# alejandrofontan/AnyFeature-VSLAM

Hardware: AMD Instinct MI355X
Metric: keypoints extracted+matched /sec (ORB32, 640x480) (higher is better)
Workload: dtype u8; 1 GPU; ORB32 640x480 synthetic corners frames (LCG), 1000 kp/frame budget, 8 levels x1.2, FAST 20; extract+describe on device, brute-force Hamming match frame t vs t-1 (TH 75, ratio 0.6, orientation check); parallelism=frames sharded x1

## Files before the change

anyfeature-vslam_amd/csrc/k_harris.hip:

```cpp
#include <algorithm>

#include "afv_device.h"
#include "afv_wave.h"
#include "afv_runtime.h"

typedef short short2v __attribute__((ext_vector_type(2)));
typedef unsigned int uint2v __attribute__((ext_vector_type(2)));
typedef unsigned int uint3v __attribute__((ext_vector_type(3)));
__device__ __forceinline__ uint32_t as_u32(short2v v) { return __builtin_bit_cast(uint32_t, v); }
__device__ __forceinline__ short2v as_s2(uint32_t v) { return __builtin_bit_cast(short2v, v); }

#define RS_CPT 36
#define HQ_CHUNK 64

__device__ __forceinline__ int wave_incl_scan_shfl(int v) { return afv_wave_incl_scan(v); }

__global__ __launch_bounds__(256) void k_retain_score(const Geo *__restrict__ geo_p, const uint32_t *__restrict__ cand_packed,
                                                      const int *__restrict__ cand_count, uint32_t *__restrict__ l1,
                                                      int *__restrict__ l1_count, uint2 *__restrict__ queue, int *__restrict__ queue_n,
                                                      int frame_base, int total_blocks) {
    __shared__ int hist[256];
    __shared__ int wsum[4];
    __shared__ int s_T1, s_n1, s_qb;
    const Geo &geo = *geo_p;
    const int work = afv_xcd_remap(blockIdx.x, total_blocks);
    if (work >= total_blocks) return;
    const int l = work % geo.nlevels, f = frame_base + work / geo.nlevels;
    const LevelGeo &L = geo.lv[l];
    const size_t base = L.cand_off + (size_t)f * L.cand_frame_stride;
    const uint32_t *cp = cand_packed + base;
    uint32_t *out = l1 + base;
    const int n = min(cand_count[f * AFV_MAX_LEVELS + l], L.cand_cap);
    const int tid = threadIdx.x, lane = tid & 63;
    const int K = 2 * L.cv_quota;
    int n1 = n;
    const bool reg = n <= 256 * RS_CPT;
    uint32_t cpk[RS_CPT];
    if (reg) {
#pragma unroll
        for (int k = 0; k < RS_CPT; ++k) {
            cpk[k] = 0;
            if (k * 256 < n && k * 256 + tid < n) cpk[k] = cp[k * 256 + tid];
        }
    }
    if (n > K) {
        hist[tid] = 0;
        if (tid == 0) {
            s_T1 = 0;
            s_n1 = 0;
        }
        __syncthreads();
        if (reg) {
#pragma unroll
            for (int k = 0; k < RS_CPT; ++k)
                if (k * 256 < n && k * 256 + tid < n) atomicAdd(&hist[cpk[k] >> 24], 1);
        } else {
            for (int i = tid; i < n; i += 256) atomicAdd(&hist[cp[i] >> 24], 1);
        }
        __syncthreads();
        const int h = hist[255 - tid];
        const int incl = wave_incl_scan_shfl(h);
        if (lane == 63) wsum[tid >> 6] = incl;
        __syncthreads();
        int before = incl - h;
        for (int w = 0; w < (tid >> 6); ++w) before += wsum[w];
        if (before < K && K <= before + h) s_T1 = 255 - tid;
        __syncthreads();
        const int T1 = s_T1;
        auto emit = [&](bool in, uint32_t e) {
            const bool keep = in && (int)(e >> 24) >= T1;
            const unsigned long long m = __ballot(keep);
            int wbase = 0;
            if (lane == 0 && m) wbase = atomicAdd(&s_n1, __popcll(m));
            wbase = __shfl(wbase, 0, 64);
            if (keep) out[wbase + __popcll(m & ((1ull << lane) - 1ull))] = e;
        };
        if (reg) {
#pragma unroll
            for (int k = 0; k < RS_CPT; ++k) {
                if (k * 256 >= n) break;
                emit(k * 256 + tid < n, cpk[k]);
            }
        } else {
            for (int i0 = 0; i0 < n; i0 += 256) {
                const int i = i0 + tid;
                emit(i < n, i < n ? cp[i] : 0u);
            }
        }
        __syncthreads();
        n1 = s_n1;
    } else if (reg) {
#pragma unroll
        for (int k = 0; k < RS_CPT; ++k)
            if (k * 256 < n && k * 256 + tid < n) out[k * 256 + tid] = cpk[k];
    } else {
        for (int i = tid; i < n; i += 256) out[i] = cp[i];
    }
    const int nchunks = (n1 + HQ_CHUNK - 1) / HQ_CHUNK;
    if (tid == 0) {
        l1_count[f * AFV_MAX_LEVELS + l] = n1;
        s_qb = nchunks ? atomicAdd(queue_n, nchunks) : 0;
    }
    __syncthreads();
    const int qb = s_qb;
    for (int i = tid; i < nchunks; i += 256) queue[qb + i] = make_uint2((uint32_t)(f * AFV_MAX_LEVELS + l), (uint32_t)(i * HQ_CHUNK) | ((uint32_t)min(HQ_CHUNK, n1 - i * HQ_CHUNK) << 24));
}

struct HarrisItem {
    const uint8_t *img;
    __amdgpu_buffer_rsrc_t rsrc;
    int pitch, lw, lh, cnt;
    size_t base;
};

__device__ __forceinline__ void harris_item_rsrc(HarrisItem &it) {
    const uint64_t ip = reinterpret_cast<uint64_t>(it.img);
    const uint32_t ip_lo = (uint32_t)__builtin_amdgcn_readfirstlane((int)(uint32_t)ip), ip_hi = (uint32_t)__builtin_amdgcn_readfirstlane((int)(uint32_t)(ip >> 32));
    it.img = reinterpret_cast<const uint8_t *>(((uint64_t)ip_hi << 32) | ip_lo);
    it.pitch = __builtin_amdgcn_readfirstlane(it.pitch);
    it.lw = __builtin_amdgcn_readfirstlane(it.lw);
    it.lh = __builtin_amdgcn_readfirstlane(it.lh);
    it.rsrc = __builtin_amdgcn_make_buffer_rsrc(const_cast<uint8_t *>(it.img), 0, (it.lh - 1) * it.pitch + it.lw, 0x00027000);
}

__device__ __forceinline__ HarrisItem harris_item(const Geo &geo, const FrameSrc &src0, const uint8_t *pyr, uint2 item) {
    HarrisItem it;
    const int fl = (int)item.x, f = fl / AFV_MAX_LEVELS, l = fl - f * AFV_MAX_LEVELS;
    const LevelGeo &L = geo.lv[l];
    if (l == 0) {
        it.img = src0.base + (size_t)f * src0.frame_stride;
        it.pitch = src0.stride;
    } else {
        it.img = pyr + L.pyr_off + (size_t)f * L.pyr_frame_stride;
        it.pitch = L.pitch;
    }
    it.lw = L.w;
    it.lh = L.h;
    it.cnt = (int)(item.y >> 24);
    it.base = L.cand_off + (size_t)f * L.cand_frame_stride + (size_t)(item.y & 0x00ffffffu);
    harris_item_rsrc(it);
    return it;
}

__device__ __forceinline__ float harris_response(const HarrisItem &it, uint32_t e, float scale4) {
    const int px = (int)(e & 4095u), py = (int)((e >> 12) & 4095u);
    const bool left = px < 4, right = px + 4 >= it.lw;
    const int xa = left ? 0 : ((px - 4) & ~3), sh = left ? 0 : ((px - 4) & 3);
    const uint32_t selA = 0x0c010c00u + (uint32_t)sh * 0x00010001u, selB = selA + 0x00020002u;
    const uint32_t selC = (right ? 0x0c0c0c02u : 0x0c0c0c04u) + (uint32_t)sh;
    uint32_t off[9];
    off[1] = (uint32_t)(py - 3) * (uint32_t)it.pitch + (uint32_t)xa;
#pragma unroll
    for (int r = 2; r < 8; ++r) off[r] = off[r - 1] + (uint32_t)it.pitch;
    off[0] = (py == 3) ? off[2] : off[1] - (uint32_t)it.pitch;
    off[8] = (py + 4 >= it.lh) ? off[6] : off[7] + (uint32_t)it.pitch;
    uint32_t w[9][3];
#pragma unroll
    for (int r = 0; r < 9; ++r) {
        const uint3v v = __builtin_amdgcn_raw_buffer_load_b96(it.rsrc, off[r], 0, 0);
        w[r][0] = v.x;
        w[r][1] = v.y;
        w[r][2] = v.z;
    }
    if (py + 5 >= it.lh && xa + 12 > it.lw) {
#pragma unroll
        for (int r = 6; r < 9; ++r) {
            const uint2v v = __builtin_amdgcn_raw_buffer_load_b64(it.rsrc, off[r], 0, 0);
            uint32_t w2 = 0;
            for (int j = 0; j < 4; ++j)
                if (xa + 8 + j < it.lw) w2 |= (uint32_t)it.img[off[r] + 8 + j] << (8 * j);
            w[r][0] = v.x;
            w[r][1] = v.y;
            w[r][2] = w2;
        }
    }
    if (left) {
#pragma unroll
        for (int r = 0; r < 9; ++r) {
            w[r][2] = __builtin_amdgcn_alignbit(w[r][2], w[r][1], 24);
            w[r][1] = __builtin_amdgcn_alignbit(w[r][1], w[r][0], 24);
            w[r][0] = (w[r][0] << 8) | ((w[r][0] >> 8) & 0xffu);
        }
    }
    short2v two;
    two.x = two.y = 2;
    short2v P[3][5];
    int a = 0, b = 0, c = 0;
#pragma unroll
    for (int r = 0; r < 9; ++r) {
        short2v *row = P[r % 3];
        row[0] = as_s2(__builtin_amdgcn_perm(w[r][1], w[r][0], selA));
        row[1] = as_s2(__builtin_amdgcn_perm(w[r][1], w[r][0], selB));
        row[2] = as_s2(__builtin_amdgcn_perm(w[r][2], w[r][1], selA));
        row[3] = as_s2(__builtin_amdgcn_perm(w[r][2], w[r][1], selB));
        row[4] = as_s2(__builtin_amdgcn_perm(w[r][2], w[r][1], selC));
        if (r >= 2) {
            const short2v *r0 = P[(r - 2) % 3], *r1 = P[(r - 1) % 3], *r2 = row;
            short2v Sp[5], Dp[5];
#pragma unroll
            for (int k = 0; k < 5; ++k) {
                Sp[k] = r1[k] * two + r0[k] + r2[k];
                Dp[k] = r2[k] - r0[k];
            }
#pragma unroll
            for (int k = 0; k < 4; ++k) {
                short2v Ix = Sp[k + 1] - Sp[k];
                const short2v O = as_s2(__builtin_amdgcn_alignbit(as_u32(Dp[k + 1]), as_u32(Dp[k]), 16));
                short2v Iy = O * two + Dp[k] + Dp[k + 1];
                if (k == 3) {
                    Ix = as_s2(as_u32(Ix) & 0xffffu);
                    Iy = as_s2(as_u32(Iy) & 0xffffu);
                }
                a = __builtin_amdgcn_sdot2(Ix, Ix, a, false);
                b = __builtin_amdgcn_sdot2(Iy, Iy, b, false);
                c = __builtin_amdgcn_sdot2(Ix, Iy, c, false);
            }
        }
    }
    const float fa = (float)a, fb = (float)b, fc = (float)c;
    const float sum = fa + fb;
    return ((fa * fb - fc * fc) - (0.04f * sum) * sum) * scale4;
}

__global__ __launch_bounds__(256) void k_harris(const Geo *__restrict__ geo_p, FrameSrc src0, const uint8_t *__restrict__ pyr,
                                                const uint32_t *__restrict__ l1, float *__restrict__ l1_resp,
                                                const uint2 *__restrict__ queue, const int *__restrict__ queue_n) {
    const Geo &geo = *geo_p;
    const int qn = *queue_n;
    const int lane = threadIdx.x & 63;
    const int nwaves = (int)gridDim.x * 4;
    const int wv = __builtin_amdgcn_readfirstlane(afv_xcd_remap((int)blockIdx.x, (int)gridDim.x) * 4 + (int)(threadIdx.x >> 6));
    const int per = (qn + nwaves - 1) / nwaves;
    const int w_end = min(qn, (wv + 1) * per);
    for (int w = wv * per; w < w_end; ++w) {
        const HarrisItem it = harris_item(geo, src0, pyr, queue[w]);
        if (lane < it.cnt) l1_resp[it.base + lane] = harris_response(it, l1[it.base + lane], geo.harris_scale4);
    }
}

#define RH_T 1024
#define RH_SLICES 4
#define RH_CPT 12
#define RH_SURV 3072

template <bool REG>
__device__ __forceinline__ void retain_harris_small_body(const Geo &geo, const FrameSrc &src0, const uint8_t *__restrict__ pyr,
                                                         const uint32_t *__restrict__ cp, int n, int l, int f, int slice, size_t base,
                                                         uint32_t *__restrict__ l1, int *__restrict__ l1_count, float *__restrict__ l1_resp) {
    __shared__ int hist[4][256];
    __shared__ int wsum[4];
    __shared__ int s_T1, s_before, s_mine;
    __shared__ uint32_t s_surv[RH_SURV];
    const LevelGeo &L = geo.lv[l];
    const int tid = threadIdx.x, lane = tid & 63;
    const int K = 2 * L.cv_quota;
    const int start = (int)((long)n * slice / RH_SLICES), end = (int)((long)n * (slice + 1) / RH_SLICES);
    const int nk = (n + RH_T - 1) / RH_T;
    uint32_t cpk[RH_CPT];
    if (REG) {
#pragma unroll
        for (int k = 0; k < RH_CPT; ++k) cpk[k] = (k < nk && k * RH_T + tid < n) ? cp[k * RH_T + tid] : 0u;
    }
#define RH_FOR_ITEMS(BODY)                                            \
    if (REG) {                                                        \
        _Pragma("unroll") for (int k = 0; k < RH_CPT; ++k) {          \
            const int i = k * RH_T + tid;                             \
            const uint32_t e = cpk[k];                                \
            if (k < nk) { BODY }                                      \
        }                                                             \
    } else {                                                          \
        for (int k = 0; k < nk; ++k) {                                \
            const int i = k * RH_T + tid;                             \
            const uint32_t e = i < n ? cp[i] : 0u;                    \
            { BODY }                                                  \
        }                                                             \
    }
    int T1 = 0;
    if (tid == 0) {
        s_before = 0;
        s_mine = 0;
    }
    if (n > K) {
        if (tid < 256) hist[0][tid] = hist[1][tid] = hist[2][tid] = hist[3][tid] = 0;
        if (tid == 0) s_T1 = 0;
        __syncthreads();
        RH_FOR_ITEMS(if (i < n) atomicAdd(&hist[lane & 3][e >> 24], 1);)
        __syncthreads();
        int h = 0, incl = 0;
        if (tid < 256) {
            h = hist[0][255 - tid] + hist[1][255 - tid] + hist[2][255 - tid] + hist[3][255 - tid];
            incl = afv_wave_incl_scan(h);
            if (lane == 63) wsum[tid >> 6] = incl;
        }
        __syncthreads();
        if (tid < 256) {
            int before = incl - h;
            for (int w = 0; w < (tid >> 6); ++w) before += wsum[w];
            if (before < K && K <= before + h) s_T1 = 255 - tid;
        }
        __syncthreads();
        T1 = s_T1;
    } else {
        __syncthreads();
    }
    {
        int c = 0;
        RH_FOR_ITEMS(c += (i < start && (int)(e >> 24) >= T1) ? 1 : 0;)
        c = afv_wave_incl_scan(c);
        if (lane == 63 && c) atomicAdd(&s_before, c);
    }
    __syncthreads();
    int out_base = s_before;
    HarrisItem it;
    if (l == 0) {
        it.img = src0.base + (size_t)f * src0.frame_stride;
        it.pitch = src0.stride;
    } else {
        it.img = pyr + L.pyr_off + (size_t)f * L.pyr_frame_stride;
        it.pitch = L.pitch;
    }
    it.lw = L.w;
    it.lh = L.h;
    it.cnt = 0;
    it.base = 0;
    harris_item_rsrc(it);
    for (int s0 = start; s0 < end; s0 += RH_SURV) {
        const int s1 = min(s0 + RH_SURV, end);
        RH_FOR_ITEMS(
            if (k * RH_T < s1 && (k + 1) * RH_T > s0) {
                const bool keep = i >= s0 && i < s1 && (int)(e >> 24) >= T1;
                const unsigned long long m = __ballot(keep);
                int wbase = 0;
                if (lane == 0 && m) wbase = atomicAdd(&s_mine, __popcll(m));
                wbase = __shfl(wbase, 0, 64);
                if (keep) s_surv[wbase + __popcll(m & ((1ull << lane) - 1ull))] = e;
            })
        __syncthreads();
        const int cnt = s_mine;
        for (int j = tid; j < cnt; j += RH_T) {
            const uint32_t es = s_surv[j];
            l1[base + out_base + j] = es;
            l1_resp[base + out_base + j] = harris_response(it, es, geo.harris_scale4);
        }
        out_base += cnt;
        if (s0 + RH_SURV < end) {
            __syncthreads();
            if (tid == 0) s_mine = 0;
            __syncthreads();
        }
    }
#undef RH_FOR_ITEMS
    if (slice == RH_SLICES - 1 && tid == 0) l1_count[f * AFV_MAX_LEVELS + l] = out_base;
}

__global__ __launch_bounds__(RH_T) void k_retain_harris_small(const Geo *__restrict__ geo_p, FrameSrc src0, const uint8_t *__restrict__ pyr,
                                                              const uint32_t *__restrict__ cand_packed, const int *__restrict__ cand_count,
                                                              uint32_t *__restrict__ l1, int *__restrict__ l1_count, float *__restrict__ l1_resp,
                                                              int frame_base, int total_blocks) {
    const Geo &geo = *geo_p;
    const int work = (int)blockIdx.x;
    if (work >= total_blocks) return;
    const int slice = work % RH_SLICES, fl = work / RH_SLICES;
    const int l = fl % geo.nlevels, f = frame_base + fl / geo.nlevels;
    const LevelGeo &L = geo.lv[l];
    const size_t base = L.cand_off + (size_t)f * L.cand_frame_stride;
    const int n = min(cand_count[f * AFV_MAX_LEVELS + l], L.cand_cap);
    if (n <= RH_T * RH_CPT) retain_harris_small_body<true>(geo, src0, pyr, cand_packed + base, n, l, f, slice, base, l1, l1_count, l1_resp);
    else retain_harris_small_body<false>(geo, src0, pyr, cand_packed + base, n, l, f, slice, base, l1, l1_count, l1_resp);
}

extern "C" size_t afv_harris_queue_per_frame(const Geo *g) {
    size_t n = 0;
    for (int l = 0; l < g->nlevels; ++l) n += (size_t)(g->lv[l].cand_cap + HQ_CHUNK - 1) / HQ_CHUNK;
    return n;
}

extern "C" void afv_launch_retain_harris(const Geo *geo_dev, int nlevels, const FrameSrc *src0, const uint8_t *pyr,
                                         const uint32_t *cand_packed, const int *cand_count, uint32_t *l1, int *l1_count,
                                         float *l1_resp, uint2 *queue, int *queue_n, int frame_base, int nframes, int small, hipStream_t stream) {
    if (small) {
        const int total = nlevels * nframes * RH_SLICES;
        hipLaunchKernelGGL(k_retain_harris_small, dim3(total), dim3(RH_T), 0, stream, geo_dev, *src0, pyr, cand_packed, cand_count, l1, l1_count,
                           l1_resp, frame_base, total);
        return;
    }
    const int total = nlevels * nframes;
    hipLaunchKernelGGL(k_retain_score, dim3((total + 7) / 8 * 8), dim3(256), 0, stream, geo_dev, cand_packed, cand_count, l1, l1_count,
                       queue, queue_n, frame_base, total);
    const int grid = (int)std::min<long>(std::max<long>((long)nframes * 80, 256), 65536) & ~7;
    hipLaunchKernelGGL(k_harris, dim3(grid), dim3(256), 0, stream, geo_dev, *src0, pyr, l1, l1_resp, queue, queue_n);
}
```

Before: 224.8 million keypoints/s.

## Compact retain-score output per wave and share vertical sums in Harris

In the retain-score kernel, each wave now owns a contiguous slice of candidates. Kept entries are counted per wave and prefix-summed through shared memory, which replaces the per-iteration LDS atomic on s_n1 for the register path. In the Harris response, pairwise row sums r1+r2 are computed once and reused across the two windows that share them, so 2*r1+r0+r2 becomes T0+T1. The selector constant is also changed so the k==3 Ix mask can be dropped. Output order changes to per-wave contiguous, and the rewritten selC and masking must still produce the same Harris values.

```diff
diff --git a/anyfeature-vslam_amd/csrc/k_harris.hip b/anyfeature-vslam_amd/csrc/k_harris.hip
--- a/anyfeature-vslam_amd/csrc/k_harris.hip
+++ b/anyfeature-vslam_amd/csrc/k_harris.hip
@@ -20,7 +20,7 @@
                                                       int *__restrict__ l1_count, uint2 *__restrict__ queue, int *__restrict__ queue_n,
                                                       int frame_base, int total_blocks) {
     __shared__ int hist[256];
-    __shared__ int wsum[4];
+    __shared__ int wsum[4], wkeep[4];
     __shared__ int s_T1, s_n1, s_qb;
     const Geo &geo = *geo_p;
     const int work = afv_xcd_remap(blockIdx.x, total_blocks);
@@ -35,12 +35,16 @@
     const int K = 2 * L.cv_quota;
     int n1 = n;
     const bool reg = n <= 256 * RS_CPT;
+    const int wave = __builtin_amdgcn_readfirstlane(tid >> 6);
+    const int per_w = (n + 255) / 256 * 64;
+    const int wb = wave * per_w;
+    auto mine = [&](int k) { return k * 64 < per_w && wb + k * 64 + lane < n; };
     uint32_t cpk[RS_CPT];
     if (reg) {
 #pragma unroll
         for (int k = 0; k < RS_CPT; ++k) {
             cpk[k] = 0;
-            if (k * 256 < n && k * 256 + tid < n) cpk[k] = cp[k * 256 + tid];
+            if (mine(k)) cpk[k] = cp[wb + k * 64 + lane];
         }
     }
     if (n > K) {
@@ -53,46 +57,57 @@
         if (reg) {
 #pragma unroll
             for (int k = 0; k < RS_CPT; ++k)
-                if (k * 256 < n && k * 256 + tid < n) atomicAdd(&hist[cpk[k] >> 24], 1);
+                if (mine(k)) atomicAdd(&hist[cpk[k] >> 24], 1);
         } else {
             for (int i = tid; i < n; i += 256) atomicAdd(&hist[cp[i] >> 24], 1);
         }
         __syncthreads();
         const int h = hist[255 - tid];
         const int incl = wave_incl_scan_shfl(h);
-        if (lane == 63) wsum[tid >> 6] = incl;
+        if (lane == 63) wsum[wave] = incl;
         __syncthreads();
         int before = incl - h;
-        for (int w = 0; w < (tid >> 6); ++w) before += wsum[w];
+        for (int w = 0; w < wave; ++w) before += wsum[w];
         if (before < K && K <= before + h) s_T1 = 255 - tid;
         __syncthreads();
         const int T1 = s_T1;
-        auto emit = [&](bool in, uint32_t e) {
-            const bool keep = in && (int)(e >> 24) >= T1;
-            const unsigned long long m = __ballot(keep);
-            int wbase = 0;
-            if (lane == 0 && m) wbase = atomicAdd(&s_n1, __popcll(m));
-            wbase = __shfl(wbase, 0, 64);
-            if (keep) out[wbase + __popcll(m & ((1ull << lane) - 1ull))] = e;
-        };
         if (reg) {
+            auto keeps = [&](int k) { return mine(k) && (int)(cpk[k] >> 24) >= T1; };
+            int kept = 0;
+#pragma unroll
+            for (int k = 0; k < RS_CPT; ++k) kept += __popcll(__ballot(keeps(k)));
+            if (lane == 0) wkeep[wave] = kept;
+            __syncthreads();
+            int slot = 0;
+            for (int w = 0; w < wave; ++w) slot += wkeep[w];
+            n1 = wkeep[0] + wkeep[1] + wkeep[2] + wkeep[3];
 #pragma unroll
             for (int k = 0; k < RS_CPT; ++k) {
-                if (k * 256 >= n) break;
-                emit(k * 256 + tid < n, cpk[k]);
+                if (k * 64 >= per_w) break;
+                const bool keep = keeps(k);
+                const unsigned long long m = __ballot(keep);
+                const int below = (int)__builtin_amdgcn_mbcnt_hi((uint32_t)(m >> 32), __builtin_amdgcn_mbcnt_lo((uint32_t)m, 0u));
+                if (keep) out[slot + below] = cpk[k];
+                slot += __popcll(m);
             }
         } else {
             for (int i0 = 0; i0 < n; i0 += 256) {
                 const int i = i0 + tid;
-                emit(i < n, i < n ? cp[i] : 0u);
+                const uint32_t e = i < n ? cp[i] : 0u;
+                const bool keep = i < n && (int)(e >> 24) >= T1;
+                const unsigned long long m = __ballot(keep);
+                int wbase = 0;
+                if (lane == 0 && m) wbase = atomicAdd(&s_n1, __popcll(m));
+                wbase = __shfl(wbase, 0, 64);
+                if (keep) out[wbase + __popcll(m & ((1ull << lane) - 1ull))] = e;
             }
-        }
-        __syncthreads();
-        n1 = s_n1;
+            __syncthreads();
+            n1 = s_n1;
+        }
     } else if (reg) {
 #pragma unroll
         for (int k = 0; k < RS_CPT; ++k)
-            if (k * 256 < n && k * 256 + tid < n) out[k * 256 + tid] = cpk[k];
+            if (mine(k)) out[wb + k * 64 + lane] = cpk[k];
     } else {
         for (int i = tid; i < n; i += 256) out[i] = cp[i];
     }
@@ -147,7 +162,7 @@
     const bool left = px < 4, right = px + 4 >= it.lw;
     const int xa = left ? 0 : ((px - 4) & ~3), sh = left ? 0 : ((px - 4) & 3);
     const uint32_t selA = 0x0c010c00u + (uint32_t)sh * 0x00010001u, selB = selA + 0x00020002u;
-    const uint32_t selC = (right ? 0x0c0c0c02u : 0x0c0c0c04u) + (uint32_t)sh;
+    const uint32_t selC = (right ? 0x0c030c02u : 0x0c030c04u) + (uint32_t)sh * 0x00010001u;
     uint32_t off[9];
     off[1] = (uint32_t)(py - 3) * (uint32_t)it.pitch + (uint32_t)xa;
 #pragma unroll
@@ -182,9 +197,10 @@
             w[r][0] = (w[r][0] << 8) | ((w[r][0] >> 8) & 0xffu);
         }
     }
-    short2v two;
-    two.x = two.y = 2;
+    uint32_t two = 0x00020002u;
+    asm("" : "+s"(two));
     short2v P[3][5];
+    short2v T[2][5];
     int a = 0, b = 0, c = 0;
 #pragma unroll
     for (int r = 0; r < 9; ++r) {
@@ -194,23 +210,25 @@
         row[2] = as_s2(__builtin_amdgcn_perm(w[r][2], w[r][1], selA));
         row[3] = as_s2(__builtin_amdgcn_perm(w[r][2], w[r][1], selB));
         row[4] = as_s2(__builtin_amdgcn_perm(w[r][2], w[r][1], selC));
+        if (r >= 1) {
+            const short2v *r1 = P[(r - 1) % 3];
+#pragma unroll
+            for (int k = 0; k < 5; ++k) T[(r - 1) % 2][k] = r1[k] + row[k];
+        }
         if (r >= 2) {
-            const short2v *r0 = P[(r - 2) % 3], *r1 = P[(r - 1) % 3], *r2 = row;
+            const short2v *r0 = P[(r - 2) % 3], *T0 = T[r % 2], *T1 = T[(r - 1) % 2];
             short2v Sp[5], Dp[5];
 #pragma unroll
             for (int k = 0; k < 5; ++k) {
-                Sp[k] = r1[k] * two + r0[k] + r2[k];
-                Dp[k] = r2[k] - r0[k];
+                Sp[k] = T0[k] + T1[k];
+                Dp[k] = row[k] - r0[k];
             }
 #pragma unroll
             for (int k = 0; k < 4; ++k) {
-                short2v Ix = Sp[k + 1] - Sp[k];
+                const short2v Ix = Sp[k + 1] - Sp[k];
                 const short2v O = as_s2(__builtin_amdgcn_alignbit(as_u32(Dp[k + 1]), as_u32(Dp[k]), 16));
-                short2v Iy = O * two + Dp[k] + Dp[k + 1];
-                if (k == 3) {
-                    Ix = as_s2(as_u32(Ix) & 0xffffu);
-                    Iy = as_s2(as_u32(Iy) & 0xffffu);
-                }
+                short2v Iy = O * as_s2(two) + (Dp[k] + Dp[k + 1]);
+                if (k == 3) Iy = as_s2(as_u32(Iy) & 0xffffu);
                 a = __builtin_amdgcn_sdot2(Ix, Ix, a, false);
                 b = __builtin_amdgcn_sdot2(Iy, Iy, b, false);
                 c = __builtin_amdgcn_sdot2(Ix, Iy, c, false);
```

Result: no change. 225.0 million keypoints/s, median of 6 (+0.1%).
